# ZINZINBIN/Disruption-Prediciton-based-on-Multimodal-Deep-Learning

Measured on AMD Instinct MI355X. Metric: clips/sec (fwd+bwd) R2Plus1D T=21 128x128, higher is better.
Workload: dtype f32 storage; products as 3 fp16 (forward) / bf16 (backward) MFMAs on hi+lo splits, f32 accumulate; 1 GPU; R2Plus1D layer_sizes=[1,2,2,1] alpha=0.01, per-GPU clips (8,3,21,128,128) fp32, forward+FocalLoss(gamma=2)+backward+clip_grad_norm(1.0)+AdamW(2e-4), BN in train mode; per_gpu_batch=8, global_batch=8, parallelism=dp1

## Files before the change

### disruption-prediciton-based-on-multimodal-deep-learning_amd/csrc/bn_elem.hip

```cpp
#include "common.h"
#include "patch_common.h"

struct View {
  const float* p; const float* scale; const float* shift; float slope;
};
static inline View to_view(const MdActView* v) {
  View o; o.p = v ? v->data : nullptr; o.scale = v ? v->scale : nullptr; o.shift = v ? v->shift : nullptr;
  o.slope = v ? v->slope : 1.f; return o;
}

struct ChanConst { float4 sc, sh; };
__device__ __forceinline__ ChanConst load_cc(const View& v, int c4) {
  ChanConst k;
  if (v.scale) { k.sc = *(const float4*)(v.scale + c4 * 4); k.sh = *(const float4*)(v.shift + c4 * 4); }
  else { k.sc = make_float4(1.f, 1.f, 1.f, 1.f); k.sh = make_float4(0.f, 0.f, 0.f, 0.f); }
  return k;
}
__device__ __forceinline__ float4 pre_of(const View& v, const ChanConst& k, float4 x) {
  if (!v.scale) return x;
  return make_float4(fmaf(x.x, k.sc.x, k.sh.x), fmaf(x.y, k.sc.y, k.sh.y), fmaf(x.z, k.sc.z, k.sh.z), fmaf(x.w, k.sc.w, k.sh.w));
}
__device__ __forceinline__ float4 act_of(const View& v, float4 pre) {
  if (!v.scale) return pre;
  return make_float4(md_leaky(pre.x, v.slope), md_leaky(pre.y, v.slope), md_leaky(pre.z, v.slope), md_leaky(pre.w, v.slope));
// ... 19 lines not shown
  w.r = threadIdx.x / C4;
  w.active = w.r < w.nr;
  const int64_t per = (rows + gridDim.x - 1) / gridDim.x;
  w.beg = (int64_t)bid * per;
  w.end = w.beg + per < rows ? w.beg + per : rows;
  return w;
}

static int stream_blocks(int64_t rows, int C4) {
  const int nr = 256 / C4;
  int64_t b = md_cdiv64(rows, (int64_t)nr * 8);
  if (b < 1) b = 1;
  if (b > 4096) b = 4096;
  return (int)b;
}

__global__ __launch_bounds__(256) void k_bn_act(View v, int64_t rows, int C4, float* __restrict__ out) {
  RowWalk w = row_walk(rows, C4);
  if (!w.active) return;
  const ChanConst k = load_cc(v, w.c4);
  for (int64_t row = w.beg + w.r; row < w.end; row += w.nr) {
    const size_t o = ((size_t)row * C4 + w.c4) * 4;
    *(float4*)(out + o) = act_of(v, pre_of(v, k, *(const float4*)(v.p + o)));
  }
}

__global__ __launch_bounds__(256) void k_residual_fwd(View skip, View main, float alpha, int64_t rows, int C4,
                                                      float* __restrict__ z) {
  RowWalk w = row_walk(rows, C4);
  if (!w.active) return;
// ... 625 lines not shown
```

### disruption-prediciton-based-on-multimodal-deep-learning_amd/csrc/common.h

```cpp
#pragma once
#include <hip/hip_runtime.h>
#include <hip/hip_ext.h>
#include <stdint.h>
#include <tuple>
#include <type_traits>
#include <utility>
#include "../../include/mi355x_disrupt.h"

typedef float f32x4 __attribute__((ext_vector_type(4)));

#define MD_ABI_VERSION 1

static inline int md_cdiv(int a, int b) { return (a + b - 1) / b; }
static inline int64_t md_cdiv64(int64_t a, int64_t b) { return (a + b - 1) / b; }
static inline int md_round_up(int a, int b) { return md_cdiv(a, b) * b; }

struct MdProfHook { void* ctx; int (*acquire)(void* ctx, hipEvent_t* start, hipEvent_t* stop); };
extern thread_local MdProfHook g_md_prof_hook;

template <typename... P, size_t... I>
static inline void md_klaunch_fill(std::tuple<P...>& vals, void** ptrs, std::index_sequence<I...>) {
  ((ptrs[I] = (void*)&std::get<I>(vals)), ...);
}
template <typename... P, typename... A>
// ... 38 lines not shown

__device__ __forceinline__ float md_leaky(float v, float slope) {
  const float s = v * slope;
  return (slope >= 0.f && slope <= 1.f) ? fmaxf(v, s) : (v > 0.f ? v : s);
}
__device__ __forceinline__ float md_dleaky(float pre, float slope) { return pre > 0.f ? 1.f : slope; }

struct PGeom;
int linear_split_launch(int f16, const float* A, int M, int K, const float* W, int Kp, int N16, float* C, int ldc, int accumulate,
                        hipStream_t s);
struct PatchPlan;
const PatchPlan* patch_lookup(const MdConvDesc* d, int dgrad);
size_t patch_wpack_floats(const PatchPlan* p);
int patch_blocks(const PatchPlan* p);
int patch_pack(const MdConvDesc* d, int dgrad, const PatchPlan* p, const float* w, float* out, hipStream_t s);
struct PersBwd;
int patch_launch(const PatchPlan* p, const float* src, const float* ps, const float* psh, float slope, const float* wp,
                 float* dst, float* stat, int accumulate, hipStream_t s, const PersBwd* bw = nullptr);
bool patch_can_fuse(const PatchPlan* p);
int patch_fused_blocks(const PatchPlan* p);

struct WgradPlan;
extern thread_local int g_wgrad_beside;
struct WgradBeside { WgradBeside() { ++g_wgrad_beside; } ~WgradBeside() { --g_wgrad_beside; } };
const WgradPlan* wgrad_lookup(const MdConvDesc* d, int xpitch = 0, int xc0 = 0, int dw_cin = 0);
size_t wgrad_patch_workspace_floats(const WgradPlan* p);
bool wgrad_plan_xsplit_ok(const WgradPlan* p);
bool wgrad_plan_second_form(const WgradPlan* p);
int wgrad_patch_launch(const WgradPlan* p, const MdConvDesc* d, const float* src, const float* ps, const float* psh,
                       float slope, const float* dy, float* dw, float* slab, hipStream_t s, int ysplit = 0, int xsplit = 0);
// ... 14 lines not shown
```

### disruption-prediciton-based-on-multimodal-deep-learning_amd/csrc/conv_patch.hip

```cpp
#include "common.h"
#include <cstdlib>

#include "patch_common.h"

template <bool F16, int NT = 256>
__device__ __forceinline__ void stage_image(__amdgpu_buffer_rsrc_t src, int Cpitch, int c0, int cvalid4,
                                            const int* sG, int npix, int C8, unsigned magic, char* img, int pitch,
                                            int lo_off, bool prologue, const float* sScale, const float* sShift,
                                            float pslope, int t, bool presplit = false) {
  const int total = npix * C8;
  for (int base = 0; base < total; base += NT * 4) {
    float4 va[4], vb[4];
    int pix[4], c8s[4];
#pragma unroll
    for (int u = 0; u < 4; ++u) {
      const int item = min(base + u * NT + t, total - 1);
      const int pixel = mdiv(item, magic);
      const int c8 = item - pixel * C8;
      const int gp = sG[pixel];
      const bool in = gp >= 0 && c8 * 2 < cvalid4;
      const unsigned off = in ? (presplit ? (unsigned)(gp * C8 + c8) * 32u : (unsigned)(gp * Cpitch + c0 + c8 * 8) * 4u) : MD_OOB;
      va[u] = buf_load4(src, off);
      vb[u] = buf_load4(src, (in && (presplit || c8 * 2 + 1 < cvalid4)) ? off + 16u : MD_OOB);
      pix[u] = base + u * NT + t < total ? (pixel | (in ? 0 : 0x20000000)) : -1;
// ... 408 lines not shown
  g.off_pixg = (int)off; off += (size_t)((g.P * 4 + 15) & ~15);
  g.off_scale = (int)off; off += (size_t)2 * PMAXC * 4;
  if (!pers_wgs && off > cap) return false;
  if (pers_wgs && (g.pt >= 64 || g.py >= 512 || g.px >= 512 || g.bt >= 256 || g.by >= 256 || g.bx >= 256)) return false;
  if (getenv("MD_PLAN_PRINT"))
    fprintf(stderr, "patch%s %s %d->%d k%d%d%d s%d%d%d dst %dx%dx%d: box %dx%dx%d patch %dx%dx%d=%d C8=%d stages=%d lds=%zu\n",
            pers_wgs ? "(persistent)" : (pm_rows != PM ? "(half)" : ""), dgrad ? (cls ? "dgrad-class" : "dgrad") : "fwd", d->Cin, d->Cout, d->kt, d->kh, d->kw, d->st, d->sh, d->sw, g.Td, g.Hd,
            g.Wd, g.bt, g.by, g.bx, g.pt, g.py, g.px, g.P, g.C8, g.nstages, off);
  *out = g; *lds_bytes = off;
  return true;
}

#include <atomic>
static std::atomic<int> g_pers_grid{0};
extern "C" int md_set_pers_grid(int n) { return g_pers_grid.exchange(n > 0 ? n : 0); }
struct PersVariant {
  bool on; PersGeom pg; size_t lds; int grid;
  int nsl; PersGeom sl[4]; size_t sl_lds[4];
};
struct PatchClass { PGeom g; size_t lds; size_t wp_off; ClassSpec spec; PersVariant pers; };
struct PatchPlan {
  PGeom g; size_t lds; int N; int dgrad; int ncls; PatchClass cls[8]; PersVariant pers;
  bool half; PGeom gh; size_t ldsh; int half_npb;
};

static void pers_try(const MdConvDesc* d, int dgrad, const ClassSpec* cls, const PGeom& classic, PersVariant* pv) {
  pv->on = false; pv->nsl = 0;
  static const int off = getenv("MD_PERS") && atoi(getenv("MD_PERS")) == 0;
  static const int off_f = getenv("MD_PERS_FWD") && atoi(getenv("MD_PERS_FWD")) == 0;
  static const int off_d = getenv("MD_PERS_DGRAD") && atoi(getenv("MD_PERS_DGRAD")) == 0;
// ... 1 lines not shown
  static const int min_rows = getenv("MD_PERS_MIN_ROWS") ? atoi(getenv("MD_PERS_MIN_ROWS")) : 96;
  const int grid_override = g_pers_grid.load();
  PGeom g; size_t lds = 0;
  if (!patch_build(d, dgrad, &g, &lds, cls, 1)) return;
  if (g.Kc8 != classic.Kc8 || g.N16 != classic.N16 || g.nstages != classic.nstages) return;
  if (!grid_override && g.bt * g.by * g.bx < min_rows) return;
  PersGeom pg; pg.g = g;
  int grid = 0;
  if (!pers_finish(&pg, &lds, &grid)) return;
  if (grid_override) grid = grid_override;
  pg.nboxes = d->N * g.nbt * g.nby * g.nbx;
  if (pg.nboxes >= 65536 || pg.nboxes < 2 * grid) return;
  pg.nit = md_cdiv(g.P * g.C8, 256);
  if (pg.nit > PERS_MAXI || (pg.nit > 4 && g.N16 > 48) || g.N16 > 96) return;
  pg.m_nbx = magic_of(g.nbx); pg.m_nby = magic_of(g.nby); pg.m_nbt = magic_of(g.nbt);
  pv->on = true; pv->pg = pg; pv->lds = lds; pv->grid = grid;
  pv->nsl = 0;
  static const int slices_on = getenv("MD_FUSE_SLICES") && atoi(getenv("MD_FUSE_SLICES")) == 1;
  if (dgrad && slices_on && g.N16 > 48 && pg.nit <= 4) {
    int n0 = 0, k = 0; bool ok = true;
    while (n0 < g.N16 && ok) {
      const int rem = g.N16 - n0;
      const int w = (rem >= 80 || rem == 48) ? 48 : (rem > 48 ? 32 : rem);
      if (w < 32 || k >= 4) { ok = false; break; }
      PersGeom sg = pg; sg.g.N16 = w;
      size_t sl = 0; int gr = 0;
      if (!pers_finish(&sg, &sl, &gr)) { ok = false; break; }
      sg.nboxes = pg.nboxes; sg.nit = pg.nit; sg.m_nbx = pg.m_nbx; sg.m_nby = pg.m_nby; sg.m_nbt = pg.m_nbt;
      sg.n0 = n0; sg.N16w = g.N16;
      pv->sl[k] = sg; pv->sl_lds[k] = sl; ++k; n0 += w;
// ... 45 lines not shown

const PatchPlan* patch_lookup(const MdConvDesc* d, int dgrad) {
  if (g_exact_fp32.load()) return nullptr;
  {
    static const int dis_f = getenv("MD_PATCH_FWD") && atoi(getenv("MD_PATCH_FWD")) == 0;
    static const int dis_d = getenv("MD_PATCH_DGRAD") && atoi(getenv("MD_PATCH_DGRAD")) == 0;
    if ((dgrad && dis_d) || (!dgrad && dis_f)) return nullptr;
  }
  {
    static const int prefer = getenv("MD_LINEAR_PREFER") ? atoi(getenv("MD_LINEAR_PREFER")) : 1;
    if (prefer && d->kt == 1 && d->kh == 1 && d->kw == 1 && d->st == 1 && d->sh == 1 && d->sw == 1 && d->pt == 0 && d->ph == 0 && d->pw == 0 &&
        d->N == 1 && d->Ti == 1 && d->Hi == 1 && d->Wi >= 4096 && (d->Cin & 3) == 0 && (d->Cout & 3) == 0)
      return nullptr;
  }
  static std::mutex mu;
  static std::map<std::array<int, 20>, PatchPlan*> cache;
  std::array<int, 20> key = {d->N, d->Ti, d->Hi, d->Wi, d->Cin, d->To, d->Ho, d->Wo, d->Cout, d->kt, d->kh, d->kw,
                             d->st, d->sh, d->sw, d->pt, d->ph, d->pw, dgrad, g_pers_grid.load()};
  std::lock_guard<std::mutex> lock(mu);
  auto it = cache.find(key);
  if (it != cache.end()) return it->second;
  PatchPlan* pp = nullptr;
  PGeom g; size_t lds = 0;
  static const int no_cls = getenv("MD_DGRAD_CLASSES") && atoi(getenv("MD_DGRAD_CLASSES")) == 0;
  if (dgrad && !no_cls && (d->st != 1 || d->sh != 1 || d->sw != 1)) {
    PatchPlan* cp = new PatchPlan();
    cp->ncls = patch_classes(d, cp);
    if (cp->ncls > 0) { cp->g = cp->cls[0].g; cp->lds = cp->cls[0].lds; cp->N = d->N; cp->dgrad = 1; cp->pers.on = false; pp = cp; }
    else delete cp;
  }
  if (pp) pp->half = false;
  if (!pp && patch_build(d, dgrad, &g, &lds)) {
    pp = new PatchPlan(); pp->g = g; pp->lds = lds; pp->N = d->N; pp->dgrad = dgrad; pp->ncls = 0;
// ... 230 lines not shown
    case 5: LAUNCH_PATCH(F16_, STR_, 5, W8_); break;                                                                    \
    case 6: LAUNCH_PATCH(F16_, STR_, 6, W8_); break;                                                                    \
    case 7: LAUNCH_PATCH(F16_, STR_, 7, W8_); break;                                                                    \
    case 8: LAUNCH_PATCH(F16_, STR_, 8, W8_); break;                                                                    \
    default: LAUNCH_PATCH(F16_, STR_, 9, W8_); break;                                                                   \
  }
  if (!p->dgrad) { if (w8) { LAUNCH_PATCH_NR(true, false, true); } else { LAUNCH_PATCH_NR(true, false, false); } }
  else if (!g.strided) { if (w8) { LAUNCH_PATCH_NR(false, false, true); } else { LAUNCH_PATCH_NR(false, false, false); } }
  else { LAUNCH_PATCH_NR(false, true, false); }
  MD_CHECK_LAUNCH();
  return MD_OK;
}

static bool pers_can_fuse(const PersVariant& pv) {
  static const int maxn = getenv("MD_FUSE_MAXN16") ? atoi(getenv("MD_FUSE_MAXN16")) : 48;
  return pv.on && pv.pg.g.N16 <= maxn && !(pv.pg.g.N16 == 48 && pv.pg.nit > 4) && !(pv.pg.g.N16 > 48 && pv.pg.nit > 4);
}
static bool fuse_per_box(const PersVariant& pv) {
  static const int patch_off = getenv("MD_FUSE_PATCH") && atoi(getenv("MD_FUSE_PATCH")) == 0;
  static const int pers_fallback_on = getenv("MD_FUSE_PERS_FALLBACK") && atoi(getenv("MD_FUSE_PERS_FALLBACK")) == 1;
  if (patch_off) return false;
  if (!pv.on) return true;
  return !pers_can_fuse(pv) && pers_fallback_on;
}
bool patch_can_fuse(const PatchPlan* p) {
  if (!p->dgrad) return false;
  auto ok = [](const PersVariant& pv) { return pers_can_fuse(pv) || (pv.on && pv.nsl > 0) || fuse_per_box(pv); };
  if (!p->ncls) return ok(p->pers);
  for (int c = 0; c < p->ncls; ++c) if (!ok(p->cls[c].pers)) return false;
  return true;
}
// ... 154 lines not shown
```

### disruption-prediciton-based-on-multimodal-deep-learning_amd/csrc/conv_pers.hip

```cpp
#include "patch_common.h"
#include <cstdlib>
#include <cstdio>
#include <type_traits>

__device__ __forceinline__ void buf_store4(__amdgpu_buffer_rsrc_t r, unsigned off, f32x4 v) {
  __builtin_amdgcn_raw_buffer_store_b128(__builtin_bit_cast(__attribute__((__vector_size__(4 * sizeof(unsigned)))) unsigned, v), r, off, 0, 0);
}
__device__ __forceinline__ f32x4 buf_load4v(__amdgpu_buffer_rsrc_t r, unsigned off) {
  return __builtin_bit_cast(f32x4, __builtin_amdgcn_raw_buffer_load_b128(r, off, 0, 0));
}
__device__ __forceinline__ f32x4 buf_load4_pinned(__amdgpu_buffer_rsrc_t r, unsigned off) {
  return __builtin_bit_cast(f32x4, __builtin_amdgcn_raw_buffer_load_b128(r, off, 0, 0));
}

template <bool F16, bool FUSE, int NREP, int MAXI>
__global__ __launch_bounds__(512) void k_conv_pers(
    PersGeom pg, const float* __restrict__ src, const float* __restrict__ pscale, const float* __restrict__ pshift,
    float pslope, const uint4* __restrict__ wp, float* __restrict__ dst, float* __restrict__ stat_partial,
    int accumulate, PersBwd bw) {
  extern __shared__ __attribute__((aligned(16))) char sm[];
  const PGeom& g = pg.g;
  constexpr int NT = 512, TT = 256;
  const int t = threadIdx.x;
  const int wave = __builtin_amdgcn_readfirstlane(t >> 6);
  const int team = wave >> 2, wr = wave & 3;
  const int tt = t & (TT - 1);
  const int lane = t & 63, li = lane & 15, lg = lane >> 4;
  const bool prologue = pscale != nullptr;
  const bool stats = stat_partial != nullptr;
  const int dbg = (accumulate >> 8) & 0xff;
// ... 20 lines not shown
  }
  if (t < 32) ((int*)(sm + pg.off_sync))[t] = 0;
  if (t < PM) {
    const int rt = mdiv(t, g.m_byx); const int r = t - rt * g.byx;
    const int ry = mdiv(r, g.m_bx); const int rx = r - ry * g.bx;
    const bool v = rt < g.bt;
    int2 ri;
    ri.x = v ? ((rt * g.st * g.py + ry * g.sh) * g.px + rx * g.sw) * g.ppitch : 0;
    ri.y = v ? (rt | (ry << 8) | (rx << 16)) : -1;
    sRow[t] = ri;
  }
  if (prologue) for (int c = t; c < pg.sc_stride; c += NT) {
    const int cs = g.pack2 ? (c & 3) : c;
    sScale[c] = c < g.Cps ? pscale[cs] : 0.f; sShift[c] = c < g.Cps ? pshift[cs] : 0.f;
  }
  if (FUSE) {
    for (int c = t; c < g.N16; c += NT) {
      const int cg = pg.n0 + c;
      const bool ok = cg < g.Cpd;
      sBn[c] = ok ? bw.scale[cg] : 0.f; sBn[bns + c] = ok ? bw.shift[cg] : 0.f;
      sBn[2 * bns + c] = ok ? bw.mean[cg] : 0.f; sBn[3 * bns + c] = ok ? bw.invstd[cg] : 0.f;
    }
  }
  {
    const int total = g.nstages * 2 * g.N16 * 8;
    const int kchunks = pg.nsteps * 4;
    for (int idx = t; idx < total; idx += NT) {
      const int c = idx & 7; const int rest = idx >> 3;
      const int hb = rest / g.N16; const int n = rest - hb * g.N16;
      const int h = hb & 1, kb = hb >> 1;
// ... 21 lines not shown
      it_rel[u] = presplit ? (((ppt * g.Hs + ppy) * g.Ws + ppx) * g.C8 + c8) * 8 : ((ppt * g.Hs + ppy) * g.Ws + ppx) * g.Cps + c8 * 8;
      it_pd[u] = (unsigned)ppt | ((unsigned)ppy << 6) | ((unsigned)ppx << 15) | ((unsigned)c8 << 24) |
                 ((c8 * 2 < cvalid4 ? 1u : 0u) << 30) | ((c8 * 2 + 1 < cvalid4 ? 1u : 0u) << 31);
    }
  }
  const int rp0 = sRow[wr * 32 + li].x, rp1 = sRow[wr * 32 + 16 + li].x;
  int rdec[2], drel[2];
#pragma unroll
  for (int a = 0; a < 2; ++a) {
    const int pk = sRow[wr * 32 + a * 16 + li].y;
    rdec[a] = pk;
    const int rt = pk & 0xff, ry = (pk >> 8) & 0xff, rx = (pk >> 16) & 0xff;
    drel[a] = pk < 0 ? 0 : ((rt * g.dmt * g.Hdf) + ry * g.dmh) * g.Wdf + rx * g.dmw;
  }
  const int c0 = lg * 4;
  f32x4 s1[NREP], s2[NREP];
#pragma unroll
  for (int j = 0; j < NREP; ++j) { s1[j] = (f32x4){0.f, 0.f, 0.f, 0.f}; s2[j] = s1[j]; }

  const __amdgpu_buffer_rsrc_t srs = make_rsrc(src, presplit ? (unsigned)(g.src_bytes / (g.Cps * 4u)) * (unsigned)g.C8 * 32u : g.src_bytes);
  const __amdgpu_buffer_rsrc_t drs = make_rsrc(dst, g.dst_bytes);
  const __amdgpu_buffer_rsrc_t yrs = make_rsrc(FUSE ? bw.yraw : dst, g.dst_bytes);

  f32x4 va[MAXI], vb[MAXI];
  unsigned inmask = 0;
  auto issue = [&](int box) {
    int b = box;
    const int q1 = mdiv(b, pg.m_nbx); const int xb = b - q1 * g.nbx; b = q1;
    const int q2 = mdiv(b, pg.m_nby); const int yb = b - q2 * g.nby; b = q2;
    const int n = mdiv(b, pg.m_nbt); const int tb = b - n * g.nbt;
    const int ot = tb * g.bt * g.st + g.org_t, oh = yb * g.by * g.sh + g.org_h, ow = xb * g.bx * g.sw + g.org_w;
    const int qbase = (((n * g.Ts + ot) * g.Hs + oh) * g.Ws + ow) * (presplit ? g.C8 * 8 : g.Cps);
    inmask = 0;
// ... 139 lines not shown
      for (int j = 0; j < YD; ++j) request_y(j);
    }
    if (nxt < pg.nboxes && !(dbg & 8)) commit();
    if (early_issue && nxt + stride < pg.nboxes) issue(nxt + stride);
    if (cur < pg.nboxes && !(dbg & 32)) {
      const bool allin = __all(gw[0] != 0.f && gw[1] != 0.f);
#pragma unroll
      for (int j = 0; j < NREP; ++j) {
        if constexpr (FUSE) { if (j + YD < NREP) { request_y(j + YD); __builtin_amdgcn_sched_barrier(0); } }
        const bool colok = pg.n0 + c0 + j * 16 < g.Cpd;
#pragma unroll
        for (int a = 0; a < 2; ++a) {
          const unsigned off = (colok && !(dbg & 4)) ? goff[a] + j * 64u : MD_OOB;
          f32x4 v = acc[a][j];
          if (accumulate) v += buf_load4v(drs, off);
          if constexpr (FUSE) {
            const f32x4 sc = *(const f32x4*)(sBn + c0 + j * 16), sh = *(const f32x4*)(sBn + bns + c0 + j * 16);
            const f32x4 mu = *(const f32x4*)(sBn + 2 * bns + c0 + j * 16), is = *(const f32x4*)(sBn + 3 * bns + c0 + j * 16);
            const f32x4 y = yv[j][a];
#pragma unroll
            for (int r = 0; r < 4; ++r) {
              const float pre = fmaf(y[r], sc[r], sh[r]);
              v[r] *= md_dleaky(pre, bw.slope);
              const float gm = v[r] * gw[a];
              s1[j][r] += gm; s2[j][r] = fmaf(gm, (y[r] - mu[r]) * is[r], s2[j][r]);
            }
          } else if (stats) {
            if (allin) {
#pragma unroll
              for (int r = 0; r < 4; ++r) { s1[j][r] += v[r]; s2[j][r] = fmaf(v[r], v[r], s2[j][r]); }
            } else {
// ... 29 lines not shown
      while (__hip_atomic_load(ctr, __ATOMIC_RELAXED, __HIP_MEMORY_SCOPE_WORKGROUP) < target) __builtin_amdgcn_s_sleep(2);
      __builtin_amdgcn_fence(__ATOMIC_ACQUIRE, "workgroup");
    };
    while (cur < pg.nboxes) {
      do_matrix();
      team_sync();
      do_move();
      team_sync();
      cur += stride;
    }
    __syncthreads();
  }
#endif

  if (stats) {
    float* red = (float*)(sm + pg.off_red);
#pragma unroll
    for (int j = 0; j < NREP; ++j)
#pragma unroll
      for (int r = 0; r < 4; ++r) {
        float a1 = s1[j][r], a2 = s2[j][r];
#pragma unroll
        for (int m = 1; m < 16; m <<= 1) { a1 += __shfl_xor(a1, m); a2 += __shfl_xor(a2, m); }
        if (li == 0) {
          red[(wave * 2 + 0) * (PNREP * 16) + c0 + j * 16 + r] = a1;
          red[(wave * 2 + 1) * (PNREP * 16) + c0 + j * 16 + r] = a2;
        }
      }
    __syncthreads();
    if (t < g.N16 && pg.n0 + t < g.Cpd) {
      float a1 = 0.f, a2 = 0.f;
#pragma unroll
      for (int w = 0; w < 8; ++w) {
        a1 += red[(w * 2 + 0) * (PNREP * 16) + t];
        a2 += red[(w * 2 + 1) * (PNREP * 16) + t];
      }
      float* sp = stat_partial + (size_t)blockIdx.x * 2 * g.Cpd + pg.n0;
      sp[t] = a1;
      sp[g.Cpd + t] = a2;
    }
  }
}

static int pers_num_cus() {
  static int n = 0;
  if (!n) {
    int dev = 0; hipDeviceProp_t p;
    if (hipGetDevice(&dev) == hipSuccess && hipGetDeviceProperties(&p, dev) == hipSuccess && p.multiProcessorCount > 0) n = p.multiProcessorCount;
    else { (void)hipGetLastError(); n = 256; }
  }
// ... 8 lines not shown
  pg->n0 = 0; pg->N16w = g.N16;
  pg->patch_bytes = (g.P * g.ppitch + 15) & ~15;
  size_t off = (size_t)2 * pg->patch_bytes;
  pg->off_red = 0;
  if (off < (size_t)8 * 2 * PNREP * 16 * 4) off = (size_t)8 * 2 * PNREP * 16 * 4;
  pg->off_bres = (int)off; off += (size_t)2 * g.N16 * pg->bpitch;
  pg->off_k = (int)off; off += (size_t)(pg->nsteps * 4 + 4) * 4;
  off = (off + 15) & ~(size_t)15;
  pg->off_row = (int)off; off += (size_t)PM * 8;
  pg->sc_stride = g.C8 * 8; pg->bn_stride = g.N16;
  pg->off_sc = (int)off; off += (size_t)2 * pg->sc_stride * 4;
  pg->off_bn = (int)off; off += (size_t)4 * pg->bn_stride * 4;
  off = (off + 15) & ~(size_t)15;
  pg->off_sync = (int)off; off += 128;
  if (off > (size_t)(160 * 1024)) return false;
  *lds_bytes = off;
  *grid = pers_num_cus();
  return true;
}

size_t pers_bres_bytes(int Kc8, int N16) {
  int u = md_cdiv(Kc8, 4) * 4; while ((u & 3) != 2) ++u;
  return (size_t)2 * N16 * u * 16;
}
size_t pers_fixed_bytes(int Cps, int N16) { return (size_t)PM * 8 + (size_t)(2 * (Cps + 8) + 4 * N16) * 4 + 256 + 144; }

int pers_launch(const PersGeom& pg, size_t lds, int grid, bool f16, const float* src, const float* ps, const float* psh, float slope,
                const float* wp, float* dst, float* stat, int accumulate, const PersBwd& bw, hipStream_t s) {
  const PGeom& g = pg.g;
  const int nrep = g.N16 / 16;
  const int nblk = pers_blocks(pg, grid);
  static const int dbg = getenv("MD_DBG") ? atoi(getenv("MD_DBG")) : 0;
// ... 16 lines not shown
    switch (nrep) {                                                                                                     \
      case 2: LAUNCH_PERS(F16_, FUSE_, 2, 8); break;                                                                    \
      case 3: LAUNCH_PERS(F16_, FUSE_, 3, 8); break;                                                                    \
      default: return MD_ERR_UNSUPPORTED;                                                                               \
    }                                                                                                                   \
  } else {                                                                                                              \
    switch (nrep) {                                                                                                     \
      case 2: LAUNCH_PERS(F16_, FUSE_, 2, 4); break;                                                                    \
      case 3: LAUNCH_PERS(F16_, FUSE_, 3, 4); break;                                                                    \
      case 4: LAUNCH_PERS(F16_, FUSE_, 4, 4); break;                                                                    \
      case 5: LAUNCH_PERS(F16_, FUSE_, 5, 4); break;                                                                    \
      case 6: LAUNCH_PERS(F16_, FUSE_, 6, 4); break;                                                                    \
      default: return MD_ERR_UNSUPPORTED;                                                                               \
    }                                                                                                                   \
  }
  if (f16) { if (bw.yraw) return MD_ERR_UNSUPPORTED; LAUNCH_PERS_NR(true, false); }
  else if (bw.yraw) { LAUNCH_PERS_NR(false, true); }
  else { LAUNCH_PERS_NR(false, false); }
  MD_CHECK_LAUNCH();
  return MD_OK;
}
```

### disruption-prediciton-based-on-multimodal-deep-learning_amd/csrc/patch_common.h

```cpp
#pragma once
#include "common.h"

typedef __bf16 bf16x8 __attribute__((ext_vector_type(8)));
typedef __bf16 bf16x2 __attribute__((ext_vector_type(2)));
typedef float f32x2 __attribute__((ext_vector_type(2)));

#define PM 128
#define PNREP 9
#define PB_PITCH 160
#define PMAXC 320

struct PGeom {
  int Ts, Hs, Ws, Cps;
  int Td, Hd, Wd, Cpd;
  int kh, kw, khw, taps;
  int org_t, org_h, org_w;
  int st, sh, sw;
  int strided;
  int dst_, dsh_, dsw_;
  int lt, lh, lw, oddmask;
  int kt, padt, padh, padw;
  int zero_off;
  int bt, by, bx, byx;
  int nbt, nby, nbx;
// ... 88 lines not shown
template <bool F16>
__device__ __forceinline__ f32x4 mma(uint4 a, uint4 b, f32x4 c) {
  if (F16) return __builtin_amdgcn_mfma_f32_16x16x32_f16(__builtin_bit_cast(f16x8, a), __builtin_bit_cast(f16x8, b), c, 0, 0, 0);
  return __builtin_amdgcn_mfma_f32_16x16x32_bf16(__builtin_bit_cast(bf16x8, a), __builtin_bit_cast(bf16x8, b), c, 0, 0, 0);
}


#define PERS_MAXI 8
struct PersGeom {
  PGeom g;
  int nboxes;
  int nsteps;
  int bpitch;
  int off_bres;
  int off_k, off_row, off_sc, off_red, off_bn, off_sync;
  int nit;
  int patch_bytes;
  int sc_stride, bn_stride;
  unsigned m_nbx, m_nby, m_nbt;
  int n0, N16w;
};
struct PersBwd {
  const float* yraw;
  const float* scale; const float* shift; const float* mean; const float* invstd;
  float slope;
};
bool pers_finish(PersGeom* pg, size_t* lds_bytes, int* grid);
static inline int pers_blocks(const PersGeom& pg, int grid) { const int need = (pg.nboxes + 1) / 2; return grid < need ? grid : need; }
size_t pers_bres_bytes(int Kc8, int N16);
size_t pers_fixed_bytes(int Cps, int N16);
int pers_launch(const PersGeom& pg, size_t lds, int grid, bool f16, const float* src, const float* ps, const float* psh, float slope,
                const float* wp, float* dst, float* stat, int accumulate, const PersBwd& bw, hipStream_t s);

#include <cstdlib>
static int pitch_for(int C8) {
  int u = C8;
  while ((u & 3) != 2) ++u;
  static const int add = getenv("MD_PITCH_ADD") ? atoi(getenv("MD_PITCH_ADD")) : 0;
  return (u + add) * 16;
}

static bool choose_box(int T, int H, int W, int kt, int kh, int kw, int st, int sh, int sw, int dgrad, int maxP, int softP,
// ... 28 lines not shown
```

### disruption-prediciton-based-on-multimodal-deep-learning_amd/csrc/plan.hip

```cpp
#include <vector>
#include <unordered_map>
#include <cstdlib>
#include <new>
#include "common.h"

extern "C" int md_bn_bwd_apply_fused(const float* dA, int g_in, const MdActView* main, const MdActView* skip, float alpha,
                                     const float* mean, const float* invstd, const float* partial, int32_t blocks, int64_t count,
                                     float* dgamma, float* dbeta, int64_t rows, int32_t C, float* d_raw, float* dS, void* stream);
extern "C" int md_stem_dgrad_supported(const MdConvDesc* d);
extern "C" int md_stem_dgrad(const MdConvDesc* d, const float* dy_raw, const float* w, float* dx, void* stream);
extern "C" int md_bn_eval_params(int32_t C, const float* gamma, const float* beta, const float* rmean, const float* rvar,
                                 float eps, float* mean, float* invstd, float* scale, float* shift, void* stream);

struct Unit {
  MdConvDesc d;
  int in_unit;
  int in_z;
  float slope;
  int stage;
  int64_t rows;
  size_t raw_off, stat_off, wf_off, wd_off;
  int Cp;
  int split;
  size_t slab_off;
// ... 439 lines not shown
        RC(md_residual_fwd(&skipv, &mainv, P->alpha, t2.rows, t2.d.Cout, ws + P->z[b.out_z].off, stream));
        RC(split_z(b.out_z, stream));
        ++next_block;
      }
    }
  }
  const ZT& zl = P->z.back();
  RC(md_avgpool_fwd(ws + zl.off, P->B, zl.C, zl.rows / P->B, feat, stream));
  return MD_OK;
}

static bool bn_fused_fin() {
  static const int on = getenv("MD_BN_FUSED_FIN") && atoi(getenv("MD_BN_FUSED_FIN")) == 1;
  return on;
}

static int unit_wgrad(MdPlan* P, float* ws, int ui, const MdActView& in, float* G, float* dw, void* s) {
  const Unit& u = P->units[ui];
  if (P->batch_reduce && !u.xsplit && !u.split) {
    WgradPending pd;
    const int rc = wgrad_partial(&u.d, in.data, in.scale, in.shift, in.slope, G, dw, ws + u.slab_off, (hipStream_t)s, &pd);
    if (rc == MD_OK) { P->pending.push_back(pd); return MD_OK; }
    if (rc != MD_ERR_UNSUPPORTED) return rc;
  }
  return md_conv_wgrad_fmt2(&u.d, &in, u.xsplit, G, u.split, dw, ws + P->slab_off, s);
}
static int flush_pending(MdPlan* P, void* s) {
  if (P->pending.empty()) return MD_OK;
  const int rc = wgrad2_reduce_batch((int)P->pending.size(), P->pending.data(), (hipStream_t)s);
  P->pending.clear();
  return rc;
}

static int unit_backward(MdPlan* P, float* ws, int ui, int gb, int dxb, int accumulate, bool bn_done,
                         const float* const* w, float* const* dw, float* const* dgamma, float* const* dbeta, void* stream) {
  const Unit& u = P->units[ui];
  float* G = ws + P->g_off[gb];
  float* st = ws + u.stat_off;
  (void)w;
  if (!bn_done) {
    MdActView mainv = unit_out_view(P, ws, ui);
    const int rb = P->red_blocks[ui];
    const bool fused_fin = bn_fused_fin() && !u.split;
    if (rb > 0) {
      if (fused_fin) {
        RC(md_bn_bwd_apply_fused(G, 1, &mainv, nullptr, 1.f, st, st + u.Cp, ws + P->part_off, rb, u.rows, dgamma[ui], dbeta[ui], u.rows,
                                 u.d.Cout, G, nullptr, stream));
      } else {
        RC(md_bn_bwd_finalize(ws + P->part_off, rb, u.d.Cout, u.rows, dgamma[ui], dbeta[ui], ws + P->coef_off, stream));
        RC(md_bn_bwd_apply_fmt(G, 1, &mainv, nullptr, 1.f, st, st + u.Cp, ws + P->coef_off, u.rows, u.d.Cout, G, u.split, nullptr, stream));
      }
      P->red_blocks[ui] = 0;
    } else {
      const int nb = md_bn_bwd_blocks(u.rows, u.d.Cout);
      RC(md_bn_bwd_reduce(G, &mainv, nullptr, 1.f, st, st + u.Cp, u.rows, u.d.Cout, ws + P->part_off, stream));
      if (fused_fin) {
        RC(md_bn_bwd_apply_fused(G, 0, &mainv, nullptr, 1.f, st, st + u.Cp, ws + P->part_off, nb, u.rows, dgamma[ui], dbeta[ui], u.rows,
                                 u.d.Cout, G, nullptr, stream));
// ... 220 lines not shown
```

### disruption-prediciton-based-on-multimodal-deep-learning_amd/src/_native.py

```python
from __future__ import annotations

import ctypes as C
import os
import threading

import torch

_HERE = os.path.dirname(os.path.abspath(__file__))
LIB_PATH = os.path.join(os.path.dirname(_HERE), "csrc", "libmi355x_disrupt.so")

c_float_p = C.POINTER(C.c_float)
c_void_p = C.c_void_p


class MdConvDesc(C.Structure):
    _fields_ = [(n, C.c_int32) for n in
                ("N", "Ti", "Hi", "Wi", "Cin", "To", "Ho", "Wo", "Cout", "kt", "kh", "kw", "st", "sh", "sw", "pt", "ph", "pw")]


class MdActView(C.Structure):
    _fields_ = [("data", c_void_p), ("scale", c_void_p), ("shift", c_void_p), ("slope", C.c_float)]


class MdTrainStepArgs(C.Structure):
# ... 6 lines not shown
                                         "workspace", "counters")] +
                [("ncounters", C.c_int32), ("opt_nchunks", C.c_int32)] +
                [(n, c_void_p) for n in ("opt_tensors", "opt_chunks", "opt_partial")] +
                [(n, C.c_float) for n in ("max_norm", "lr", "beta1", "beta2", "eps", "weight_decay")] +
                [("opt_step", C.c_int64), ("ok_flag", c_void_p)])


_P = c_void_p
_I32, _I64, _F, _SZ = C.c_int32, C.c_int64, C.c_float, C.c_size_t
_DESC, _VIEW = C.POINTER(MdConvDesc), C.POINTER(MdActView)
SIGNATURES = {
    "md_version": (C.c_int, [C.POINTER(C.c_char_p)]),
    "md_set_exact_fp32": (C.c_int, [C.c_int]),
    "md_get_exact_fp32": (C.c_int, []),
    "md_set_pers_grid": (C.c_int, [C.c_int]),
    "md_set_wgrad_form": (C.c_int, [C.c_int]),
    "md_conv_wpack_fwd_floats": (_SZ, [_DESC]),
    "md_conv_wpack_dgrad_floats": (_SZ, [_DESC]),
    "md_conv_pack_weights": (C.c_int, [_DESC, _P, _P, _P, _P]),
    "md_conv_pack_weights_batch": (C.c_int, [_I32, _P, _P, _P, _P, _P]),
    "md_conv_fwd_stat_blocks": (_I32, [_DESC]),
    "md_conv_fwd": (C.c_int, [_DESC, _VIEW, _P, _P, _P, _P]),
    "md_conv_dgrad": (C.c_int, [_DESC, _P, _P, _P, C.c_int, _P]),
    "md_conv_wgrad_workspace_floats": (_SZ, [_DESC]),
    "md_conv_wgrad": (C.c_int, [_DESC, _VIEW, _P, _P, _P, _P]),
    "md_bn_finalize": (C.c_int, [_P, _I32, _I32, _I64, _P, _P, _F, _F, _P, _P, _P, _P, _P, _P, _P]),
    "md_bn_eval_params": (C.c_int, [_I32, _P, _P, _P, _P, _F, _P, _P, _P, _P, _P]),
    "md_bn_act": (C.c_int, [_VIEW, _I64, _I32, _P, _P]),
    "md_residual_fwd": (C.c_int, [_VIEW, _VIEW, _F, _I64, _I32, _P, _P]),
    "md_bn_bwd_blocks": (_I32, [_I64, _I32]),
# ... 176 lines not shown
```

### include/mi355x_disrupt.h

```cpp
#ifndef MI355X_DISRUPT_H
#define MI355X_DISRUPT_H

#include <stddef.h>
#include <stdint.h>

#ifdef __cplusplus
extern "C" {
#endif

#define MD_OK 0
#define MD_ERR_BAD_SHAPE (-1)
#define MD_ERR_UNSUPPORTED (-2)
#define MD_ERR_WORKSPACE (-3)
#define MD_ERR_LAUNCH (-4)
#define MD_ERR_NULL (-5)

int md_version(const char** arch_out);

int md_set_exact_fp32(int on);
int md_get_exact_fp32(void);
int md_set_pers_grid(int n);
int md_set_wgrad_form(int first_form_only);

typedef struct MdConvDesc {
  int32_t N, Ti, Hi, Wi, Cin;
  int32_t To, Ho, Wo, Cout;
  int32_t kt, kh, kw;
  int32_t st, sh, sw;
  int32_t pt, ph, pw;
} MdConvDesc;

typedef struct MdActView {
  const float* data;
  const float* scale;
  const float* shift;
  float slope;
// ... 318 lines not shown
```

Before: 1413 clips/s.

## Extend fused BN-backward epilogue in persistent dgrad to wide channel counts via LDS sums

Lets the persistent dgrad convolution fuse the BN-backward/leaky-ReLU-gradient epilogue and its channel-sum reductions for layers with more than 48 output channel groups. Instead of keeping per-channel sums in registers per repetition, it reduces them across 16 lanes with DPP row rotations and accumulates into an LDS sum area, so register pressure stays bounded. This adds LDS use and extra template instantiations. It is on by default and can be disabled through an environment variable. Separately, it adds an opt-in, size-bounded fused BN-finalize path that stays off unless an environment variable is set.

```diff
diff --git a/disruption-prediciton-based-on-multimodal-deep-learning_amd/csrc/bn_elem.hip b/disruption-prediciton-based-on-multimodal-deep-learning_amd/csrc/bn_elem.hip
--- a/disruption-prediciton-based-on-multimodal-deep-learning_amd/csrc/bn_elem.hip
+++ b/disruption-prediciton-based-on-multimodal-deep-learning_amd/csrc/bn_elem.hip
@@ -57,6 +57,8 @@
   if (b > 4096) b = 4096;
   return (int)b;
 }
+
+int bn_apply_blocks(int64_t rows, int C4) { return stream_blocks(rows, C4); }
 
 __global__ __launch_bounds__(256) void k_bn_act(View v, int64_t rows, int C4, float* __restrict__ out) {
   RowWalk w = row_walk(rows, C4);
diff --git a/disruption-prediciton-based-on-multimodal-deep-learning_amd/csrc/common.h b/disruption-prediciton-based-on-multimodal-deep-learning_amd/csrc/common.h
--- a/disruption-prediciton-based-on-multimodal-deep-learning_amd/csrc/common.h
+++ b/disruption-prediciton-based-on-multimodal-deep-learning_amd/csrc/common.h
@@ -76,6 +76,7 @@
 size_t patch_wpack_floats(const PatchPlan* p);
 int patch_blocks(const PatchPlan* p);
 int patch_pack(const MdConvDesc* d, int dgrad, const PatchPlan* p, const float* w, float* out, hipStream_t s);
+int bn_apply_blocks(int64_t rows, int C4);
 struct PersBwd;
 int patch_launch(const PatchPlan* p, const float* src, const float* ps, const float* psh, float slope, const float* wp,
                  float* dst, float* stat, int accumulate, hipStream_t s, const PersBwd* bw = nullptr);
diff --git a/disruption-prediciton-based-on-multimodal-deep-learning_amd/csrc/conv_patch.hip b/disruption-prediciton-based-on-multimodal-deep-learning_amd/csrc/conv_patch.hip
--- a/disruption-prediciton-based-on-multimodal-deep-learning_amd/csrc/conv_patch.hip
+++ b/disruption-prediciton-based-on-multimodal-deep-learning_amd/csrc/conv_patch.hip
@@ -446,6 +446,13 @@
 #include <atomic>
 static std::atomic<int> g_pers_grid{0};
 extern "C" int md_set_pers_grid(int n) { return g_pers_grid.exchange(n > 0 ? n : 0); }
+static std::atomic<int> g_fuse_wide{-1};
+extern "C" int md_set_fuse_wide(int on) { return g_fuse_wide.exchange(on < 0 ? -1 : (on ? 1 : 0)); }
+static int fuse_wide_on() {
+  static const int env_off = getenv("MD_FUSE_PERS_WIDE") && atoi(getenv("MD_FUSE_PERS_WIDE")) == 0;
+  const int v = g_fuse_wide.load();
+  return v < 0 ? !env_off : v;
+}
 struct PersVariant {
   bool on; PersGeom pg; size_t lds; int grid;
   int nsl; PersGeom sl[4]; size_t sl_lds[4];
@@ -477,6 +484,7 @@
   pg.nit = md_cdiv(g.P * g.C8, 256);
   if (pg.nit > PERS_MAXI || (pg.nit > 4 && g.N16 > 48) || g.N16 > 96) return;
   pg.m_nbx = magic_of(g.nbx); pg.m_nby = magic_of(g.nby); pg.m_nbt = magic_of(g.nbt);
+  if (dgrad && fuse_wide_on() && g.N16 > 48 && pg.nit <= 4) (void)pers_add_sum_rows(&pg, &lds);
   pv->on = true; pv->pg = pg; pv->lds = lds; pv->grid = grid;
   pv->nsl = 0;
   static const int slices_on = getenv("MD_FUSE_SLICES") && atoi(getenv("MD_FUSE_SLICES")) == 1;
@@ -552,9 +560,9 @@
       return nullptr;
   }
   static std::mutex mu;
-  static std::map<std::array<int, 20>, PatchPlan*> cache;
-  std::array<int, 20> key = {d->N, d->Ti, d->Hi, d->Wi, d->Cin, d->To, d->Ho, d->Wo, d->Cout, d->kt, d->kh, d->kw,
-                             d->st, d->sh, d->sw, d->pt, d->ph, d->pw, dgrad, g_pers_grid.load()};
+  static std::map<std::array<int, 21>, PatchPlan*> cache;
+  std::array<int, 21> key = {d->N, d->Ti, d->Hi, d->Wi, d->Cin, d->To, d->Ho, d->Wo, d->Cout, d->kt, d->kh, d->kw,
+                             d->st, d->sh, d->sw, d->pt, d->ph, d->pw, dgrad, g_pers_grid.load(), fuse_wide_on()};
   std::lock_guard<std::mutex> lock(mu);
   auto it = cache.find(key);
   if (it != cache.end()) return it->second;
@@ -815,7 +823,9 @@
 
 static bool pers_can_fuse(const PersVariant& pv) {
   static const int maxn = getenv("MD_FUSE_MAXN16") ? atoi(getenv("MD_FUSE_MAXN16")) : 48;
-  return pv.on && pv.pg.g.N16 <= maxn && !(pv.pg.g.N16 == 48 && pv.pg.nit > 4) && !(pv.pg.g.N16 > 48 && pv.pg.nit > 4);
+  if (!pv.on) return false;
+  if (pv.pg.g.N16 > 48) return pv.pg.off_sum >= 0 && pv.pg.nit <= 4;
+  return pv.pg.g.N16 <= maxn && !(pv.pg.g.N16 == 48 && pv.pg.nit > 4);
 }
 static bool fuse_per_box(const PersVariant& pv) {
   static const int patch_off = getenv("MD_FUSE_PATCH") && atoi(getenv("MD_FUSE_PATCH")) == 0;
diff --git a/disruption-prediciton-based-on-multimodal-deep-learning_amd/csrc/conv_pers.hip b/disruption-prediciton-based-on-multimodal-deep-learning_amd/csrc/conv_pers.hip
--- a/disruption-prediciton-based-on-multimodal-deep-learning_amd/csrc/conv_pers.hip
+++ b/disruption-prediciton-based-on-multimodal-deep-learning_amd/csrc/conv_pers.hip
@@ -13,7 +13,14 @@
   return __builtin_bit_cast(f32x4, __builtin_amdgcn_raw_buffer_load_b128(r, off, 0, 0));
 }
 
-template <bool F16, bool FUSE, int NREP, int MAXI>
+__device__ __forceinline__ float row_sum16(float v) {
+#define MD_ROR(x, n) __builtin_bit_cast(float, __builtin_amdgcn_update_dpp(0, __builtin_bit_cast(int, x), 0x120 + (n), 0xf, 0xf, false))
+  v += MD_ROR(v, 8); v += MD_ROR(v, 4); v += MD_ROR(v, 2); v += MD_ROR(v, 1);
+#undef MD_ROR
+  return v;
+}
+
+template <bool F16, int FUSE, int NREP, int MAXI>
 __global__ __launch_bounds__(512) void k_conv_pers(
     PersGeom pg, const float* __restrict__ src, const float* __restrict__ pscale, const float* __restrict__ pshift,
     float pslope, const uint4* __restrict__ wp, float* __restrict__ dst, float* __restrict__ stat_partial,
@@ -64,6 +71,10 @@
     const int cs = g.pack2 ? (c & 3) : c;
     sScale[c] = c < g.Cps ? pscale[cs] : 0.f; sShift[c] = c < g.Cps ? pshift[cs] : 0.f;
   }
+  constexpr bool LSUM = FUSE == 2;
+  constexpr int SREP = LSUM ? 1 : NREP;
+  float* sSum = (float*)(sm + pg.off_sum) + wave * 2 * g.N16;
+  if (LSUM) for (int c = t; c < 8 * 2 * g.N16; c += NT) ((float*)(sm + pg.off_sum))[c] = 0.f;
   if (FUSE) {
     for (int c = t; c < g.N16; c += NT) {
       const int cg = pg.n0 + c;
@@ -115,9 +126,9 @@
     drel[a] = pk < 0 ? 0 : ((rt * g.dmt * g.Hdf) + ry * g.dmh) * g.Wdf + rx * g.dmw;
   }
   const int c0 = lg * 4;
-  f32x4 s1[NREP], s2[NREP];
-#pragma unroll
-  for (int j = 0; j < NREP; ++j) { s1[j] = (f32x4){0.f, 0.f, 0.f, 0.f}; s2[j] = s1[j]; }
+  f32x4 s1[SREP], s2[SREP];
+#pragma unroll
+  for (int j = 0; j < SREP; ++j) { s1[j] = (f32x4){0.f, 0.f, 0.f, 0.f}; s2[j] = s1[j]; }
 
   const __amdgpu_buffer_rsrc_t srs = make_rsrc(src, presplit ? (unsigned)(g.src_bytes / (g.Cps * 4u)) * (unsigned)g.C8 * 32u : g.src_bytes);
   const __amdgpu_buffer_rsrc_t drs = make_rsrc(dst, g.dst_bytes);
@@ -287,7 +298,28 @@
           const unsigned off = (colok && !(dbg & 4)) ? goff[a] + j * 64u : MD_OOB;
           f32x4 v = acc[a][j];
           if (accumulate) v += buf_load4v(drs, off);
-          if constexpr (FUSE) {
+          if constexpr (LSUM) {
+            const f32x4 sc = *(const f32x4*)(sBn + c0 + j * 16), sh = *(const f32x4*)(sBn + bns + c0 + j * 16);
+            const f32x4 mu = *(const f32x4*)(sBn + 2 * bns + c0 + j * 16), is = *(const f32x4*)(sBn + 3 * bns + c0 + j * 16);
+            const f32x4 y = yv[j][a];
+            if (a == 0) { s1[0] = (f32x4){0.f, 0.f, 0.f, 0.f}; s2[0] = s1[0]; }
+#pragma unroll
+            for (int r = 0; r < 4; ++r) {
+              const float pre = fmaf(y[r], sc[r], sh[r]);
+              v[r] *= md_dleaky(pre, bw.slope);
+              const float gm = v[r] * gw[a];
+              s1[0][r] += gm; s2[0][r] = fmaf(gm, (y[r] - mu[r]) * is[r], s2[0][r]);
+            }
+            if (a == 1) {
+              f32x4 r1, r2;
+#pragma unroll
+              for (int r = 0; r < 4; ++r) { r1[r] = row_sum16(s1[0][r]); r2[r] = row_sum16(s2[0][r]); }
+              if (li == 0) {
+                f32x4* p1 = (f32x4*)(sSum + c0 + j * 16); f32x4* p2 = (f32x4*)(sSum + g.N16 + c0 + j * 16);
+                *p1 += r1; *p2 += r2;
+              }
+            }
+          } else if constexpr (FUSE != 0) {
             const f32x4 sc = *(const f32x4*)(sBn + c0 + j * 16), sh = *(const f32x4*)(sBn + bns + c0 + j * 16);
             const f32x4 mu = *(const f32x4*)(sBn + 2 * bns + c0 + j * 16), is = *(const f32x4*)(sBn + 3 * bns + c0 + j * 16);
             const f32x4 y = yv[j][a];
@@ -347,26 +379,29 @@
 #endif
 
   if (stats) {
-    float* red = (float*)(sm + pg.off_red);
-#pragma unroll
-    for (int j = 0; j < NREP; ++j)
-#pragma unroll
-      for (int r = 0; r < 4; ++r) {
-        float a1 = s1[j][r], a2 = s2[j][r];
-#pragma unroll
-        for (int m = 1; m < 16; m <<= 1) { a1 += __shfl_xor(a1, m); a2 += __shfl_xor(a2, m); }
-        if (li == 0) {
-          red[(wave * 2 + 0) * (PNREP * 16) + c0 + j * 16 + r] = a1;
-          red[(wave * 2 + 1) * (PNREP * 16) + c0 + j * 16 + r] = a2;
+    float* red = (float*)(sm + (LSUM ? pg.off_sum : pg.off_red));
+    const int rs = LSUM ? g.N16 : PNREP * 16;
+    if constexpr (!LSUM) {
+#pragma unroll
+      for (int j = 0; j < NREP; ++j)
+#pragma unroll
+        for (int r = 0; r < 4; ++r) {
+          float a1 = s1[j][r], a2 = s2[j][r];
+#pragma unroll
+          for (int m = 1; m < 16; m <<= 1) { a1 += __shfl_xor(a1, m); a2 += __shfl_xor(a2, m); }
+          if (li == 0) {
+            red[(wave * 2 + 0) * rs + c0 + j * 16 + r] = a1;
+            red[(wave * 2 + 1) * rs + c0 + j * 16 + r] = a2;
+          }
         }
-      }
+    }
     __syncthreads();
     if (t < g.N16 && pg.n0 + t < g.Cpd) {
       float a1 = 0.f, a2 = 0.f;
 #pragma unroll
       for (int w = 0; w < 8; ++w) {
-        a1 += red[(w * 2 + 0) * (PNREP * 16) + t];
-        a2 += red[(w * 2 + 1) * (PNREP * 16) + t];
+        a1 += red[(w * 2 + 0) * rs + t];
+        a2 += red[(w * 2 + 1) * rs + t];
       }
       float* sp = stat_partial + (size_t)blockIdx.x * 2 * g.Cpd + pg.n0;
       sp[t] = a1;
@@ -405,8 +440,16 @@
   off = (off + 15) & ~(size_t)15;
   pg->off_sync = (int)off; off += 128;
   if (off > (size_t)(160 * 1024)) return false;
+  pg->off_sum = -1;
   *lds_bytes = off;
   *grid = pers_num_cus();
+  return true;
+}
+
+bool pers_add_sum_rows(PersGeom* pg, size_t* lds_bytes) {
+  const size_t off = (*lds_bytes + 15) & ~(size_t)15, need = (size_t)8 * 2 * pg->g.N16 * 4;
+  if (off + need > (size_t)(160 * 1024)) return false;
+  pg->off_sum = (int)off; *lds_bytes = off + need;
   return true;
 }
 
@@ -453,9 +496,27 @@
       default: return MD_ERR_UNSUPPORTED;                                                                               \
     }                                                                                                                   \
   }
-  if (f16) { if (bw.yraw) return MD_ERR_UNSUPPORTED; LAUNCH_PERS_NR(true, false); }
-  else if (bw.yraw) { LAUNCH_PERS_NR(false, true); }
-  else { LAUNCH_PERS_NR(false, false); }
+  if (f16) { if (bw.yraw) return MD_ERR_UNSUPPORTED; LAUNCH_PERS_NR(true, 0); }
+  else if (bw.yraw) {
+    if (nrep <= 3) {
+      switch (nrep * 2 + (pg.nit > 4)) {
+        case 4: LAUNCH_PERS(false, 1, 2, 4); break;
+        case 5: LAUNCH_PERS(false, 1, 2, 8); break;
+        case 6: LAUNCH_PERS(false, 1, 3, 4); break;
+        case 7: LAUNCH_PERS(false, 1, 3, 8); break;
+        default: return MD_ERR_UNSUPPORTED;
+      }
+    } else {
+      if (pg.nit > 4 || pg.off_sum < 0) return MD_ERR_UNSUPPORTED;
+      switch (nrep) {
+        case 4: LAUNCH_PERS(false, 2, 4, 4); break;
+        case 5: LAUNCH_PERS(false, 2, 5, 4); break;
+        case 6: LAUNCH_PERS(false, 2, 6, 4); break;
+        default: return MD_ERR_UNSUPPORTED;
+      }
+    }
+  }
+  else { LAUNCH_PERS_NR(false, 0); }
   MD_CHECK_LAUNCH();
   return MD_OK;
 }
diff --git a/disruption-prediciton-based-on-multimodal-deep-learning_amd/csrc/patch_common.h b/disruption-prediciton-based-on-multimodal-deep-learning_amd/csrc/patch_common.h
--- a/disruption-prediciton-based-on-multimodal-deep-learning_amd/csrc/patch_common.h
+++ b/disruption-prediciton-based-on-multimodal-deep-learning_amd/csrc/patch_common.h
@@ -126,6 +126,7 @@
   int bpitch;
   int off_bres;
   int off_k, off_row, off_sc, off_red, off_bn, off_sync;
+  int off_sum;
   int nit;
   int patch_bytes;
   int sc_stride, bn_stride;
@@ -138,6 +139,7 @@
   float slope;
 };
 bool pers_finish(PersGeom* pg, size_t* lds_bytes, int* grid);
+bool pers_add_sum_rows(PersGeom* pg, size_t* lds_bytes);
 static inline int pers_blocks(const PersGeom& pg, int grid) { const int need = (pg.nboxes + 1) / 2; return grid < need ? grid : need; }
 size_t pers_bres_bytes(int Kc8, int N16);
 size_t pers_fixed_bytes(int Cps, int N16);
diff --git a/disruption-prediciton-based-on-multimodal-deep-learning_amd/csrc/plan.hip b/disruption-prediciton-based-on-multimodal-deep-learning_amd/csrc/plan.hip
--- a/disruption-prediciton-based-on-multimodal-deep-learning_amd/csrc/plan.hip
+++ b/disruption-prediciton-based-on-multimodal-deep-learning_amd/csrc/plan.hip
@@ -477,6 +477,10 @@
   static const int on = getenv("MD_BN_FUSED_FIN") && atoi(getenv("MD_BN_FUSED_FIN")) == 1;
   return on;
 }
+static bool bn_fused_fin_small(int rb, int64_t rows, int Cp) {
+  static const long long bound = getenv("MD_BN_FUSED_FIN_SMALL") ? atoll(getenv("MD_BN_FUSED_FIN_SMALL")) : 0;
+  return bound > 0 && (long long)rb * bn_apply_blocks(rows, Cp / 4) * Cp <= bound;
+}
 
 static int unit_wgrad(MdPlan* P, float* ws, int ui, const MdActView& in, float* G, float* dw, void* s) {
   const Unit& u = P->units[ui];
@@ -504,7 +508,7 @@
   if (!bn_done) {
     MdActView mainv = unit_out_view(P, ws, ui);
     const int rb = P->red_blocks[ui];
-    const bool fused_fin = bn_fused_fin() && !u.split;
+    const bool fused_fin = !u.split && (bn_fused_fin() || (rb > 0 && bn_fused_fin_small(rb, u.rows, u.Cp)));
     if (rb > 0) {
       if (fused_fin) {
         RC(md_bn_bwd_apply_fused(G, 1, &mainv, nullptr, 1.f, st, st + u.Cp, ws + P->part_off, rb, u.rows, dgamma[ui], dbeta[ui], u.rows,
diff --git a/disruption-prediciton-based-on-multimodal-deep-learning_amd/src/_native.py b/disruption-prediciton-based-on-multimodal-deep-learning_amd/src/_native.py
--- a/disruption-prediciton-based-on-multimodal-deep-learning_amd/src/_native.py
+++ b/disruption-prediciton-based-on-multimodal-deep-learning_amd/src/_native.py
@@ -44,6 +44,7 @@
     "md_set_exact_fp32": (C.c_int, [C.c_int]),
     "md_get_exact_fp32": (C.c_int, []),
     "md_set_pers_grid": (C.c_int, [C.c_int]),
+    "md_set_fuse_wide": (C.c_int, [C.c_int]),
     "md_set_wgrad_form": (C.c_int, [C.c_int]),
     "md_conv_wpack_fwd_floats": (_SZ, [_DESC]),
     "md_conv_wpack_dgrad_floats": (_SZ, [_DESC]),
diff --git a/include/mi355x_disrupt.h b/include/mi355x_disrupt.h
--- a/include/mi355x_disrupt.h
+++ b/include/mi355x_disrupt.h
@@ -20,6 +20,7 @@
 int md_set_exact_fp32(int on);
 int md_get_exact_fp32(void);
 int md_set_pers_grid(int n);
+int md_set_fuse_wide(int on);
 int md_set_wgrad_form(int first_form_only);
 
 typedef struct MdConvDesc {
```

After: 1421 clips/s, median of 6. About the same (+0.5%).
